# leavesnight/VIEO_SLAM

Hardware: AMD Instinct MI355X
Metric: frontend+localBA frames/sec on EuRoC MH05 stereo-VIO; ATE vs ref (higher is better)
Workload: dtype u8 (extract/match) + f64 (pose optimisation)

## Files before the change

vieo_slam_amd/csrc/orb_extractor.hip:

```cpp
#include <algorithm>
#include <cmath>
#include <type_traits>
#include <vector>

#include "../../include/vieo_orb_pattern_31.h"
#include "common.h"
#include "sincosf_exact.h"
#include "wave_ops.h"

#define QT_DEVICE
#include "quadtree.inl"

#include "orb_internal.h"

namespace vieo {

#ifndef VIEO_RESIZE_ROWS
#define VIEO_RESIZE_ROWS 32
#endif
static const int kResizeRows = VIEO_RESIZE_ROWS;
#ifndef VIEO_QT_GROUPS
#define VIEO_QT_GROUPS {1, 64}
#endif

__global__ void __launch_bounds__(256, 8)
k_resize(OrbParams P, int l, ImgSet I, const short4* __restrict__ xtab,
         const short4* __restrict__ ytab, int lds_pitch) {
  extern __shared__ __attribute__((aligned(16))) uint8_t smem[];
  const LevelDesc& D = P.lv[l];
  const int b = blockIdx.z, tid = threadIdx.x, lane = tid & 63, wave = tid >> 6;
  const int dy0 = blockIdx.y * kResizeRows, dy1 = min(dy0 + kResizeRows, D.h);
  const int dx0 = blockIdx.x * 256, dx1 = min(dx0 + 256, D.w);
  int spitch;
  const uint8_t* src = plane_ptr(P, I, b, l - 1, &spitch);
  const short4* xt = xtab + D.xtab_off;
  const short4* yt = ytab + D.ytab_off;
  const int sy_lo = yt[dy0].x, nrows = yt[dy1 - 1].y - sy_lo + 1;
  const int sx_lo = xt[dx0].x & ~3, ndw = ((xt[dx1 - 1].y + 4) >> 2) - (sx_lo >> 2);
  {
    unsigned v[12][2];
#pragma unroll
    for (int k = 0; k < 12; k++) {
      const int r = wave + 4 * k;
      const unsigned* row = (const unsigned*)(src + (size_t)(sy_lo + r) * spitch + sx_lo);
      if (r < nrows && lane < ndw) v[k][0] = row[lane];
      if (r < nrows && lane + 64 < ndw) v[k][1] = row[lane + 64];
    }
#pragma unroll
    for (int k = 0; k < 12; k++) {
      const int r = wave + 4 * k;
      if (r < nrows && lane < ndw) *(unsigned*)(smem + r * lds_pitch + 4 * lane) = v[k][0];
      if (r < nrows && lane + 64 < ndw) *(unsigned*)(smem + r * lds_pitch + 4 * (lane + 64)) = v[k][1];
    }
    for (int r = wave; r < nrows; r += 4) {
      const unsigned* row = (const unsigned*)(src + (size_t)(sy_lo + r) * spitch + sx_lo);
      for (int c = lane + (r < 48 ? 128 : 0); c < ndw; c += 64) *(unsigned*)(smem + r * lds_pitch + 4 * c) = row[c];
    }
  }
  __syncthreads();
  const int dx4 = dx0 + lane * 4;
  if (dx4 >= D.w) return;
  int x0[4], x1[4], a0[4], a1[4];
  unsigned keep = 0;
#pragma unroll
  for (int j = 0; j < 4; j++) {
    const short4 t = xt[min(dx4 + j, D.w - 1)];
    x0[j] = t.x - sx_lo, x1[j] = t.y - sx_lo, a0[j] = t.z, a1[j] = t.w;
    if (dx4 + j < D.w) keep |= 0xFFu << (8 * j);
  }
  uint8_t* dst = I.pyr + (size_t)b * I.pyr_img + D.off;
  const int wave_u = __builtin_amdgcn_readfirstlane(wave);
  for (int dy = dy0 + wave_u; dy < dy1; dy += 4) {
    const short4 y = yt[dy];
    const uint8_t* r0 = smem + (y.x - sy_lo) * lds_pitch;
    const uint8_t* r1 = smem + (y.y - sy_lo) * lds_pitch;
    const int b0 = y.z, b1 = y.w;
    unsigned out = 0;
#pragma unroll
    for (int j = 0; j < 4; j++) {
      const int h0 = r0[x0[j]] * a0[j] + r0[x1[j]] * a1[j];
      const int h1 = r1[x0[j]] * a0[j] + r1[x1[j]] * a1[j];
      const int v = (((b0 * (int)(unsigned short)(h0 >> 4)) >> 16) + ((b1 * (int)(unsigned short)(h1 >> 4)) >> 16) + 2) >> 2;
      out |= (unsigned)(v & 0xFF) << (8 * j);
    }
    *(unsigned*)(dst + (size_t)dy * D.pitch + dx4) = out & keep;
  }
}

static const int kR2W = 200, kR2H = 26, kR2Rows = 36;
__global__ void __launch_bounds__(256, 4)
k_resize2(OrbParams P, int l, ImgSet I, const short4* __restrict__ xtab, const short4* __restrict__ ytab, int lds_pitch,
          int l1_off) {
  extern __shared__ __attribute__((aligned(16))) uint8_t smem[];
  uint8_t* l1 = smem + l1_off;
  constexpr int kL1P = 260;
  const LevelDesc& D1 = P.lv[l];
  const LevelDesc& D2 = P.lv[l + 1];
  const int b = blockIdx.z, tid = threadIdx.x, lane = tid & 63, wave = tid >> 6;
  const short4* xt1 = xtab + D1.xtab_off;
  const short4* yt1 = ytab + D1.ytab_off;
  const short4* xt2 = xtab + D2.xtab_off;
  const short4* yt2 = ytab + D2.ytab_off;
  const int ex0 = blockIdx.x * kR2W, ex1 = min(ex0 + kR2W, D2.w);
  const int ey0 = blockIdx.y * kR2H, ey1 = min(ey0 + kR2H, D2.h);
  const bool last_x = ex1 == D2.w, last_y = ey1 == D2.h;
  const int rx0 = blockIdx.x == 0 ? 0 : (xt2[ex0].x & ~3), rx1 = last_x ? D1.w : min((int)xt2[ex1 - 1].y + 1, D1.w);
  const int ry0 = blockIdx.y == 0 ? 0 : (int)yt2[ey0].x, ry1 = last_y ? D1.h : min((int)yt2[ey1 - 1].y + 1, D1.h);
  const int ox1 = last_x ? D1.w : (xt2[ex1].x & ~3), oy1 = last_y ? D1.h : (int)yt2[ey1].x;
  int spitch;
  const uint8_t* src = plane_ptr(P, I, b, l - 1, &spitch);
  const int sy_lo = yt1[ry0].x, nrows = yt1[ry1 - 1].y - sy_lo + 1;
  const int sx_lo = xt1[rx0].x & ~3, ndw = ((xt1[rx1 - 1].y + 4) >> 2) - (sx_lo >> 2);
  {
    unsigned v[12][2];
#pragma unroll
    for (int k = 0; k < 12; k++) {
      const int r = wave + 4 * k;
      const unsigned* row = (const unsigned*)(src + (size_t)(sy_lo + r) * spitch + sx_lo);
      if (r < nrows && lane < ndw) v[k][0] = row[lane];
      if (r < nrows && lane + 64 < ndw) v[k][1] = row[lane + 64];
    }
#pragma unroll
    for (int k = 0; k < 12; k++) {
      const int r = wave + 4 * k;
      if (r < nrows && lane < ndw) *(unsigned*)(smem + r * lds_pitch + 4 * lane) = v[k][0];
      if (r < nrows && lane + 64 < ndw) *(unsigned*)(smem + r * lds_pitch + 4 * (lane + 64)) = v[k][1];
    }
    for (int r = wave; r < nrows; r += 4) {
      const unsigned* row = (const unsigned*)(src + (size_t)(sy_lo + r) * spitch + sx_lo);
      for (int c = lane + (r < 48 ? 128 : 0); c < ndw; c += 64) *(unsigned*)(smem + r * lds_pitch + 4 * c) = row[c];
    }
  }
  __syncthreads();
  {
    const int dx4 = rx0 + lane * 4;
    if (dx4 < rx1) {
      int x0[4], x1[4], a0[4], a1[4];
      unsigned keep = 0;
#pragma unroll
      for (int j = 0; j < 4; j++) {
        const short4 t = xt1[min(dx4 + j, D1.w - 1)];
        x0[j] = t.x - sx_lo, x1[j] = t.y - sx_lo, a0[j] = t.z, a1[j] = t.w;
        if (dx4 + j < D1.w) keep |= 0xFFu << (8 * j);
      }
      uint8_t* dst = I.pyr + (size_t)b * I.pyr_img + D1.off;
      const bool own_x = dx4 < ox1;
      const int wave_u = __builtin_amdgcn_readfirstlane(wave);
      for (int dy = ry0 + wave_u; dy < ry1; dy += 4) {
        const short4 y = yt1[dy];
        const uint8_t* r0 = smem + (y.x - sy_lo) * lds_pitch;
        const uint8_t* r1 = smem + (y.y - sy_lo) * lds_pitch;
        const int b0 = y.z, b1 = y.w;
        unsigned out = 0;
#pragma unroll
        for (int j = 0; j < 4; j++) {
          const int h0 = r0[x0[j]] * a0[j] + r0[x1[j]] * a1[j];
          const int h1 = r1[x0[j]] * a0[j] + r1[x1[j]] * a1[j];
          const int v = (((b0 * (int)(unsigned short)(h0 >> 4)) >> 16) + ((b1 * (int)(unsigned short)(h1 >> 4)) >> 16) + 2) >> 2;
          out |= (unsigned)(v & 0xFF) << (8 * j);
        }
        out &= keep;
        *(unsigned*)(l1 + (dy - ry0) * kL1P + 4 * lane) = out;
        if (own_x && dy < oy1) *(unsigned*)(dst + (size_t)dy * D1.pitch + dx4) = out;
      }
    }
  }
  __syncthreads();
  const int dx4 = ex0 + lane * 4;
  if (dx4 >= ex1) return;
  int x0[4], x1[4], a0[4], a1[4];
  unsigned keep = 0;
#pragma unroll
  for (int j = 0; j < 4; j++) {
    const short4 t = xt2[min(dx4 + j, D2.w - 1)];
    x0[j] = t.x - rx0, x1[j] = t.y - rx0, a0[j] = t.z, a1[j] = t.w;
    if (dx4 + j < D2.w) keep |= 0xFFu << (8 * j);
  }
  uint8_t* dst2 = I.pyr + (size_t)b * I.pyr_img + D2.off;
  const int wave_u = __builtin_amdgcn_readfirstlane(wave);
  for (int dy = ey0 + wave_u; dy < ey1; dy += 4) {
    const short4 y = yt2[dy];
    const uint8_t* r0 = l1 + (y.x - ry0) * kL1P;
    const uint8_t* r1 = l1 + (y.y - ry0) * kL1P;
    const int b0 = y.z, b1 = y.w;
    unsigned out = 0;
#pragma unroll
    for (int j = 0; j < 4; j++) {
      const int h0 = r0[x0[j]] * a0[j] + r0[x1[j]] * a1[j];
      const int h1 = r1[x0[j]] * a0[j] + r1[x1[j]] * a1[j];
      const int v = (((b0 * (int)(unsigned short)(h0 >> 4)) >> 16) + ((b1 * (int)(unsigned short)(h1 >> 4)) >> 16) + 2) >> 2;
      out |= (unsigned)(v & 0xFF) << (8 * j);
    }
    *(unsigned*)(dst2 + (size_t)dy * D2.pitch + dx4) = out & keep;
  }
}

#ifndef VIEO_XCD_RUN
#define VIEO_XCD_RUN 32
#endif
static const int kXcdRun = VIEO_XCD_RUN;
__device__ __forceinline__ int xcd_grouped(int bid, int G) {
  const int xcd = bid & 7, q = bid >> 3;
  return ((q / G) * 8 + xcd) * G + q % G;
}

__device__ __forceinline__ int min3i(int a, int b, int c) { return min(min(a, b), c); }
__device__ __forceinline__ int max3i(int a, int b, int c) { return max(max(a, b), c); }

__device__ __forceinline__ int fast_strength(const uint8_t* t, int p) {
  const int v = t[0];
  int d[16];
  d[0] = v - t[3 * p];
  d[1] = v - t[3 * p + 1];
  d[2] = v - t[2 * p + 2];
  d[3] = v - t[p + 3];
  d[4] = v - t[3];
  d[5] = v - t[-p + 3];
  d[6] = v - t[-2 * p + 2];
  d[7] = v - t[-3 * p + 1];
  d[8] = v - t[-3 * p];
  d[9] = v - t[-3 * p - 1];
  d[10] = v - t[-2 * p - 2];
  d[11] = v - t[-p - 3];
  d[12] = v - t[-3];
  d[13] = v - t[p - 3];
  d[14] = v - t[2 * p - 2];
  d[15] = v - t[3 * p - 1];
  int lo3[16], hi3[16];
#pragma unroll
  for (int k = 0; k < 16; k++) {
    lo3[k] = min3i(d[k], d[(k + 1) & 15], d[(k + 2) & 15]);
    hi3[k] = max3i(d[k], d[(k + 1) & 15], d[(k + 2) & 15]);
  }
  int A = -256, B = 256;
#pragma unroll
  for (int k = 0; k < 16; k++) {
    A = max(A, min3i(lo3[k], lo3[(k + 3) & 15], lo3[(k + 6) & 15]));
    B = min(B, max3i(hi3[k], hi3[(k + 3) & 15], hi3[(k + 6) & 15]));
  }
  return max(max(A, -B), 0);
}

#ifdef VIEO_FAST_STATS
__device__ unsigned long long g_fast_stats[8];
#define FAST_STAT(i, v) do { if (lane == 0) atomicAdd(&g_fast_stats[i], (unsigned long long)(v)); } while (0)
#else
#define FAST_STAT(i, v) do { } while (0)
// ... 1055 lines not shown
    }
    D.cell_end = (int)e->cells.size();
    max_ncell = std::max(max_ncell, D.cell_end - D.cell_begin);
    D.ncap = std::max(D.nfeat, 4 * D.nIni) + 8;
    ncap_max = std::max(ncap_max, D.ncap);
    D.sel_off = sel_off;
    sel_off += D.ncap;
    if (l > 0) {
      std::vector<short> t;
      D.xtab_off = (int)(xtab.size() / 4);
      resize_axis_table(P.lv[l - 1].w, D.w, true, t);
      xtab.insert(xtab.end(), t.begin(), t.end());
      D.ytab_off = (int)(ytab.size() / 4);
      resize_axis_table(P.lv[l - 1].h, D.h, false, t);
      ytab.insert(ytab.end(), t.begin(), t.end());
      const short* xt = xtab.data() + 4 * (size_t)D.xtab_off;
      const short* yt = ytab.data() + 4 * (size_t)D.ytab_off;
      for (int y0 = 0; y0 < D.h; y0 += kResizeRows)
        resize_rows = std::max(resize_rows, yt[4 * (std::min(y0 + kResizeRows, D.h) - 1) + 1] - yt[4 * y0] + 1);
      for (int x0 = 0; x0 < D.w; x0 += 256)
        resize_dw = std::max(resize_dw, ((xt[4 * (std::min(x0 + 256, D.w) - 1) + 1] + 4) >> 2) - (xt[4 * x0] >> 2));
    }
    D.tile_begin = (int)e->tiles.size();
    D.tiles_x = (D.w + kBlurTW - 1) / kBlurTW;
    for (int ty = 0; ty < (D.h + kBlurTH - 1) / kBlurTH; ty++)
      for (int tx = 0; tx < D.tiles_x; tx++) e->tiles.push_back({(short)l, (short)tx, (short)ty, 0});
    D.tile_end = (int)e->tiles.size();
  }
  P.ncells = (int)e->cells.size();
  if (max_cw - 6 > 64 || max_ch - 6 > 1023) {
    set_error("FAST cell wider than 64 pixels (image narrower than one 30-pixel cell?)");
    return VIEO_E_INVALID;
  }
  P.cell_cap = std::max(16, ((max_cw - 6 + 1) / 2) * ((max_ch - 6 + 1) / 2));
  for (int l = 0; l < e->nlevels; l++) {
    LevelDesc& D = P.lv[l];
    D.key_off = key_off;
    D.key_cap = (D.cell_end - D.cell_begin) * P.cell_cap;
    key_off += D.key_cap;
    if (D.key_cap >= (1 << 24)) {
      set_error("too many candidate keys per level");
      return VIEO_E_INVALID;
    }
  }
  P.keys_per_image = key_off;
  P.sel_per_image = sel_off;
  P.kp_cap = sel_off;
  e->ncap_max = ncap_max;
  e->scap_max = std::max(2 * ncap_max, max_ncell);
  e->pyr_img = align_up_sz(pyr_off, 256);
  e->blur_img = align_up_sz(blur_off, 256);
  e->resize_pitch = 4 * resize_dw + 4;
  e->resize_lds = resize_rows * e->resize_pitch;
  {
    bool ok = e->nlevels >= 3;
    int rows2 = 1, dw2 = 1;
    for (int l = 1; ok && l + 1 < e->nlevels; l += 2) {
      const LevelDesc &D1 = P.lv[l], &D2 = P.lv[l + 1];
      const short* xt1 = xtab.data() + 4 * (size_t)D1.xtab_off;
      const short* yt1 = ytab.data() + 4 * (size_t)D1.ytab_off;
      const short* xt2 = xtab.data() + 4 * (size_t)D2.xtab_off;
      const short* yt2 = ytab.data() + 4 * (size_t)D2.ytab_off;
      for (int ex0 = 0; ok && ex0 < D2.w; ex0 += kR2W) {
        const int ex1 = std::min(ex0 + kR2W, D2.w);
        const int rx0 = ex0 == 0 ? 0 : (xt2[4 * ex0] & ~3), rx1 = ex1 == D2.w ? D1.w : std::min(xt2[4 * (ex1 - 1) + 1] + 1, D1.w);
        const int ox1 = ex1 == D2.w ? D1.w : (xt2[4 * ex1] & ~3);
        const int ndw = ((xt1[4 * (rx1 - 1) + 1] + 4) >> 2) - ((xt1[4 * rx0] & ~3) >> 2);
        ok = rx1 - rx0 <= 256 && ox1 <= rx1 && ox1 > rx0 && ndw <= 128;
        dw2 = std::max(dw2, ndw);
      }
      for (int ey0 = 0; ok && ey0 < D2.h; ey0 += kR2H) {
        const int ey1 = std::min(ey0 + kR2H, D2.h);
        const int ry0 = ey0 == 0 ? 0 : yt2[4 * ey0], ry1 = ey1 == D2.h ? D1.h : std::min(yt2[4 * (ey1 - 1) + 1] + 1, D1.h);
        const int oy1 = ey1 == D2.h ? D1.h : yt2[4 * ey1];
        const int nrows = yt1[4 * (ry1 - 1) + 1] - yt1[4 * ry0] + 1;
        ok = ry1 - ry0 <= kR2Rows && oy1 <= ry1 && oy1 > ry0 && nrows <= 48;
        rows2 = std::max(rows2, nrows);
      }
    }
    e->resize2_ok = ok;
    e->resize2_pitch = 4 * dw2 + 4;
    e->resize2_l1_off = (rows2 * e->resize2_pitch + 15) & ~15;
    e->resize2_lds = e->resize2_l1_off + kR2Rows * 260;
  }
  e->tpitch = align_up(max_cw + 3, 4) + 4;
  e->tile_bytes = align_up(e->tpitch * max_ch, 16);
  e->score_bytes = align_up((max_cw - 4) * (max_ch - 4), 16) + 16;
  e->fast_cand_cap = std::max(256, std::min((max_cw - 6) * (max_ch - 6), 512));
  if (const char* cc = getenv("VIEO_FAST_CAND_CAP")) e->fast_cand_cap = std::max(256, atoi(cc));
  e->fast_lds = e->tile_bytes + e->score_bytes + align_up(2 * e->fast_cand_cap, 16) + 16;
  std::vector<CellPlan> plans(e->cells.size());
  for (size_t i = 0; i < e->cells.size(); i++) {
    const CellDesc& c = e->cells[i];
    const LevelDesc& D = P.lv[c.level];
    CellPlan& p = plans[i];
    memset(&p, 0, sizeof(p));
    const int x0a = c.x0 & ~3, xo = c.x0 - x0a;
    const int ndw = ((c.x0 + c.cw + 3) >> 2) - (x0a >> 2);
    if (c.level == 0) p.off = x0a, p.row = c.y0, p.pitch = 0;
    else p.off = D.off + c.y0 * D.pitch + x0a, p.row = 0, p.pitch = D.pitch;
    p.rows = c.ch | ndw << 16 | (ndw > 16 || c.ch > 64 || c.ch < 4 ? 1 << 24 : 0);
    p.tail_toff = (c.ch - 4) * e->tpitch;
    p.kbase = (3 + c.offx) | (3 + c.offy) << 12;
    const int vw = c.cw - 6, vh = c.ch - 6;
    if (vw > 0 && vh > 0) {
      const int ng = (vw + 3) >> 2, qy = 64 / ng, rx = 64 - qy * ng, m = (4096 + ng - 1) / ng;
      p.view = vw | vh << 16;
      p.align = xo | ((3 + xo) & 3) << 8 | ((3 + xo) >> 2) << 16 | ng << 24;
      p.split = qy | rx << 8 | m << 16;
      p.G = ng * vh;
      p.step_off = qy * e->tpitch + 4 * rx;
      p.wrap_off = e->tpitch - 4 * ng;
      p.Htail = (unsigned)(0x80808080ull & ((1ull << (8 * (vw - 4 * (ng - 1)))) - 1ull));
      p.clear = ((vh + 2) * (vw + 2) + 15) / 16 | (vw + 2) << 16;
    }
  }
  if (P.ncells > 1) {
    int L = 1;
    while ((1 << L) < P.ncells) L++;
    e->cell_div_mul = (unsigned)((((unsigned long long)1 << (31 + L)) + P.ncells - 1) / P.ncells);
    e->cell_div_shift = L - 1;
  } else {
    e->cell_div_mul = 0, e->cell_div_shift = 0;
  }
  e->qt_lds = 16 * e->scap_max + (4 + 16 + 4 + 4 + 4) * ncap_max + 64 + (2 * 4 + 8 + 2 * 6) * ncap_max +
              ncap_max + 64;
  int rc;
#define ENS(buf, bytes)                 \
  if ((rc = (buf).ensure(bytes)) != VIEO_OK) return rc
  ENS(e->d_pyr, e->pyr_img * B);
  if (!orb_fused()) ENS(e->d_blur, e->blur_img * B);
  ENS(e->d_cells, plans.size() * sizeof(CellPlan));
  ENS(e->d_tiles, e->tiles.size() * sizeof(BlurTile));
  ENS(e->d_xtab, std::max<size_t>(xtab.size() * 2, 8));
  ENS(e->d_ytab, std::max<size_t>(ytab.size() * 2, 8));
  ENS(e->d_cell_keys, (size_t)B * P.ncells * P.cell_cap * 4);
  ENS(e->d_cell_counts, (size_t)B * P.ncells * 4);
  ENS(e->d_keys, (size_t)B * P.keys_per_image * 4);
  ENS(e->d_kslot, (size_t)B * P.keys_per_image * 2);
  ENS(e->d_kq, (size_t)B * P.keys_per_image);
  ENS(e->d_sel, (size_t)B * P.sel_per_image * 4);
  ENS(e->d_sel_count, (size_t)B * kMaxLevels * 4);
  ENS(e->d_tmp_kp, (size_t)B * P.kp_cap * sizeof(vieo_keypoint));
  ENS(e->d_tmp_desc, (size_t)B * P.kp_cap * 32);
  ENS(e->d_tmp_counts, (size_t)B * 2 * 4);
  ENS(e->d_krec, (size_t)B * P.kp_cap * 8);
#undef ENS
  VIEO_HIP_CHECK(hipMemcpyAsync(e->d_cells.p, plans.data(), plans.size() * sizeof(CellPlan),
                                hipMemcpyHostToDevice, e->stream));
  VIEO_HIP_CHECK(hipMemcpyAsync(e->d_tiles.p, e->tiles.data(), e->tiles.size() * sizeof(BlurTile),
                                hipMemcpyHostToDevice, e->stream));
  if (!xtab.empty()) {
    VIEO_HIP_CHECK(hipMemcpyAsync(e->d_xtab.p, xtab.data(), xtab.size() * 2, hipMemcpyHostToDevice,
                                  e->stream));
    VIEO_HIP_CHECK(hipMemcpyAsync(e->d_ytab.p, ytab.data(), ytab.size() * 2, hipMemcpyHostToDevice,
                                  e->stream));
  }
  VIEO_HIP_CHECK(hipStreamSynchronize(e->stream));
  if (e->qt_lds > 64 * 1024)
    VIEO_HIP_CHECK(hipFuncSetAttribute((const void*)k_quadtree,
                                       hipFuncAttributeMaxDynamicSharedMemorySize, e->qt_lds));
  if (e->qt_lds > 160 * 1024) {
    set_error("nfeatures too large for the LDS quadtree (%d bytes)", e->qt_lds);
    return VIEO_E_INVALID;
  }
  e->w = w;
  e->h = h;
  e->B = B;
  return VIEO_OK;
}

static int run_batch(vieo_orb* e, const uint8_t* d_images, int B, int w, int h, int stride,
                     size_t image_pitch, const int* lapping, vieo_keypoint* d_kp, uint8_t* d_desc,
                     int capacity, int32_t* d_counts) {
  int rc;
  if (w != e->w || h != e->h || B > e->B) {
    if ((rc = plan_geometry(e, w, h, std::max(B, (w == e->w && h == e->h) ? e->B : 0))) != VIEO_OK)
      return rc;
  }
  if ((stride & 3) || ((uintptr_t)d_images & 3) || (image_pitch & 3)) {
    set_error("device images need 4-byte aligned base, stride and pitch");
    return VIEO_E_INVALID;
  }
  const OrbParams& P = e->P;
  ImgSet I;
  I.img0 = d_images;
  I.stride0 = stride;
  I.img_pitch = image_pitch;
  I.pyr = e->d_pyr.as<uint8_t>();
  I.pyr_img = e->pyr_img;
  I.blur = e->d_blur.as<uint8_t>();
  I.blur_img = e->blur_img;
  e->last_imgs = I;
  e->last_B = B;
  hipStream_t st = e->stream;
  Timing& T = e->tm;
  int evi = 0;
  hipEvent_t* evs = T.ev[T.steps % kTimingRing];
#define STAMP()                                                  \
  if (T.on) VIEO_HIP_CHECK(hipEventRecord(evs[evi++], st))
  STAMP();
  static const bool resize_pairs = [] {
    const char* v = getenv("VIEO_RESIZE_PAIRS");
    return !(v && atoi(v) == 0);
  }();
  for (int l = 1; l < P.nlevels;) {
    if (resize_pairs && e->resize2_ok && (l & 1) && l + 1 < P.nlevels) {
      const LevelDesc& D2 = P.lv[l + 1];
      dim3 grd((D2.w + kR2W - 1) / kR2W, (D2.h + kR2H - 1) / kR2H, B);
      hipLaunchKernelGGL(k_resize2, grd, dim3(256), e->resize2_lds, st, P, l, I, e->d_xtab.as<short4>(), e->d_ytab.as<short4>(),
                         e->resize2_pitch, e->resize2_l1_off);
      l += 2;
      continue;
    }
    const LevelDesc& D = P.lv[l];
    dim3 grd((D.w + 255) / 256, (D.h + kResizeRows - 1) / kResizeRows, B);
    hipLaunchKernelGGL(k_resize, grd, dim3(256), e->resize_lds, st, P, l, I, e->d_xtab.as<short4>(),
                       e->d_ytab.as<short4>(), e->resize_pitch);
    l++;
  }
  STAMP();
  const auto xcd_grid = [](long long items) {
    return (unsigned)((items + 8 * kXcdRun - 1) / (8 * kXcdRun) * (8 * kXcdRun));
  };
  if ((long long)P.ncells * B > 0x7FFF0000LL || (long long)e->tiles.size() * B > 0x7FFF0000LL) {
    set_error("batch too large for one launch");
    return VIEO_E_CAPACITY;
  }
  hipLaunchKernelGGL(k_fast, dim3(xcd_grid(((long long)P.ncells * B + VIEO_FAST_WAVES - 1) / VIEO_FAST_WAVES)), dim3(64 * VIEO_FAST_WAVES),
                     (size_t)align_up(e->fast_lds, 16) * VIEO_FAST_WAVES, st, I,
                     e->d_cells.as<CellPlan>(), e->d_cell_keys.as<unsigned>(), e->d_cell_counts.as<int>(),
                     e->iniTh, e->minTh, e->tpitch, e->tile_bytes, e->score_bytes, e->fast_cand_cap, P.ncells * B, P.ncells,
                     P.cell_cap, e->cell_div_mul, e->cell_div_shift, (int)align_up(e->fast_lds, 16));
  STAMP();
  {
    static const int bounds_batch[] = VIEO_QT_GROUPS;
    static const int bounds_one[] = {64};
    const bool batch = B >= 32;
    const int* bounds = batch ? bounds_batch : bounds_one;
    const size_t n_bounds = batch ? sizeof(bounds_batch) / sizeof(bounds_batch[0]) : 1;
    auto qt_caps = [&](int la, int lb, int* ncap, int* scap) {
      int nc = 1, mc = 1;
      for (int l = la; l < lb; l++) nc = std::max(nc, P.lv[l].ncap), mc = std::max(mc, P.lv[l].cell_end - P.lv[l].cell_begin);
      *ncap = nc, *scap = std::max(2 * nc, mc);
    };
    int la = 0;
    static const int qt_env = [] {
      const char* e = getenv("VIEO_QT_THREADS");
      const int v = e ? atoi(e) : 0;
      return v > 0 ? std::min(std::max(v / 64 * 64, 64), 1024) : 0;
    }();
    const int qt_threads = qt_env > 0 ? qt_env : (B <= 16 ? 512 : 256);
    for (size_t gi = 0; gi < n_bounds && la < P.nlevels; gi++) {
      const int lb = std::min(bounds[gi], P.nlevels);
      if (lb <= la) continue;
      int nc, sc;
      qt_caps(la, lb, &nc, &sc);
      const size_t lds = (size_t)16 * sc + (4 + 16 + 4 + 4 + 4) * nc + 64 + (2 * 4 + 8 + 2 * 6) * nc + nc + 64;
      hipLaunchKernelGGL(k_quadtree, dim3(lb - la, B), dim3(qt_threads), lds, st, P,
                         e->d_cell_keys.as<unsigned>(), e->d_cell_counts.as<int>(),
                         e->d_keys.as<unsigned>(), e->d_kslot.as<unsigned short>(),
                         e->d_kq.as<unsigned char>(), e->d_sel.as<unsigned>(), e->d_sel_count.as<int>(), nc, sc, la);
      la = lb;
    }
  }
  STAMP();
  const bool fused = orb_fused();
  if (!fused) {
    int rc_b = e->d_blur.ensure(e->blur_img * (size_t)e->B);
    if (rc_b != VIEO_OK) return rc_b;
    I.blur = e->d_blur.as<uint8_t>(), e->last_imgs = I;
// ... 89 lines not shown
    for (v = 0; v <= kHalfPatch; v++) e->umax[v] = 0;
    for (v = 0; v <= vmax; ++v) e->umax[v] = cv_round_d(sqrt(hp2 - v * v));
    for (v = kHalfPatch, v0 = 0; v >= vmin; --v) {
      while (e->umax[v0] == e->umax[v0 + 1]) ++v0;
      e->umax[v] = v0;
      ++v0;
    }
  }
  hipError_t he;
  {
    int lo = 0, hi = 0;
    if (priority > 0 && hipDeviceGetStreamPriorityRange(&lo, &hi) == hipSuccess && lo != hi)
      he = hipStreamCreateWithPriority(&e->stream, hipStreamNonBlocking, hi);
    else
      he = hipStreamCreateWithFlags(&e->stream, hipStreamNonBlocking);
  }
  if (he != hipSuccess) {
    set_error("hipStreamCreate: %s", hipGetErrorString(he));
    delete e;
    return VIEO_E_HIP;
  }
  std::vector<int> pat(256);
  for (int i = 0; i < 256; i++) {
    const signed char* p = VIEO_ORB_PATTERN_31 + i * 4;
    pat[i] = (int)((unsigned)(uint8_t)p[0] | ((unsigned)(uint8_t)p[1] << 8) |
                   ((unsigned)(uint8_t)p[2] << 16) | ((unsigned)(uint8_t)p[3] << 24));
  }
  if ((rc = e->d_pattern.ensure(1024)) != VIEO_OK) {
    delete e;
    return rc;
  }
  he = hipMemcpy(e->d_pattern.p, pat.data(), 1024, hipMemcpyHostToDevice);
  if (he != hipSuccess) {
    set_error("pattern upload: %s", hipGetErrorString(he));
    delete e;
    return VIEO_E_HIP;
  }
  for (auto& set : e->tm.ev)
    for (auto& ev : set) (void)hipEventCreate(&ev);
  *out = e;
  return VIEO_OK;
}

extern "C" {

void vieo_orb_destroy(vieo_orb* e) {
  if (!e) return;
  (void)hipStreamSynchronize(e->stream);
  DevBuf* bufs[] = {&e->d_pyr,   &e->d_blur,      &e->d_cells,    &e->d_tiles,      &e->d_xtab,
                    &e->d_ytab,  &e->d_cell_keys, &e->d_cell_counts, &e->d_keys,    &e->d_kslot,
                    &e->d_kq,    &e->d_sel,       &e->d_sel_count, &e->d_pattern,   &e->d_in,
                    &e->d_kp,    &e->d_desc,      &e->d_counts,   &e->d_tmp_kp,     &e->d_tmp_desc,
                    &e->d_tmp_counts, &e->d_krec,  &e->d_io,       &e->d_uright,     &e->d_depth,
                    &e->d_sad,   &e->g_start,     &e->g_rec,      &e->g_ang};
  for (DevBuf* b : bufs) b->release();
  e->h_in.release(), e->h_res.release(), e->h_io.release();
  for (auto& set : e->tm.ev)
    for (auto& ev : set)
      if (ev) (void)hipEventDestroy(ev);
  if (e->stream) (void)hipStreamDestroy(e->stream);
  delete e;
}

int vieo_orb_levels(const vieo_orb* e) { return e->nlevels; }
float vieo_orb_scale_factor(const vieo_orb* e) { return (float)e->scaleFactor; }
static int copy_tab(const std::vector<float>& v, float* out) {
  if (!out) return VIEO_E_INVALID;
  memcpy(out, v.data(), v.size() * sizeof(float));
  return VIEO_OK;
}
int vieo_orb_scale_factors(const vieo_orb* e, float* o) { return copy_tab(e->scale, o); }
int vieo_orb_inv_scale_factors(const vieo_orb* e, float* o) { return copy_tab(e->inv_scale, o); }
int vieo_orb_level_sigma2(const vieo_orb* e, float* o) { return copy_tab(e->sigma2, o); }
int vieo_orb_inv_level_sigma2(const vieo_orb* e, float* o) { return copy_tab(e->inv_sigma2, o); }
int vieo_orb_features_per_level(const vieo_orb* e, int* o) {
  if (!o) return VIEO_E_INVALID;
  memcpy(o, e->feats.data(), e->feats.size() * sizeof(int));
  return VIEO_OK;
}
int vieo_orb_max_keypoints(const vieo_orb* e) {
  int s = 0;
  for (int l = 0; l < e->nlevels; l++) s += std::max(e->feats[l], 16) + 8;
  return s;
}

int vieo_orb_extract_batch_device(vieo_orb* e, const uint8_t* d_images, int n_images, int width,
                                  int height, int stride, size_t image_pitch_bytes,
                                  const int* h_lapping, vieo_keypoint* d_keypoints,
                                  uint8_t* d_descriptors, int capacity, int32_t* d_counts) {
  if (!e || !d_images || n_images <= 0 || !d_keypoints || !d_descriptors || !d_counts ||
      capacity <= 0) {
    set_error("vieo_orb_extract_batch_device: invalid arguments");
    return VIEO_E_INVALID;
  }
  if (width <= 0 || height <= 0) return VIEO_E_EMPTY;
  return run_batch(e, d_images, n_images, width, height, stride, image_pitch_bytes, h_lapping,
                   d_keypoints, d_descriptors, capacity, d_counts);
}

#ifdef VIEO_FAST_STATS
int vieo_fast_stats(unsigned long long* out8) {
  unsigned long long z[8] = {0};
  VIEO_HIP_CHECK(hipDeviceSynchronize());
  VIEO_HIP_CHECK(hipMemcpyFromSymbol(out8, HIP_SYMBOL(vieo::g_fast_stats), sizeof(z)));
  VIEO_HIP_CHECK(hipMemcpyToSymbol(HIP_SYMBOL(vieo::g_fast_stats), z, sizeof(z)));
  return VIEO_OK;
}
// ... 233 lines not shown
```

vieo_slam_amd/csrc/orb_internal.h:

```cpp
#pragma once
#include <vector>

#include "common.h"

namespace vieo {

static const int kPatchSize = 31, kHalfPatch = 15, kEdge = 19;
static const int kMaxLevels = 16;
#ifndef VIEO_BLUR_TH
#define VIEO_BLUR_TH 96
#endif
static const int kBlurTW = 64, kBlurTH = VIEO_BLUR_TH;

struct LevelDesc {
  int w, h, pitch, off;
  int boff;
  int cell_begin, cell_end;
  int nfeat;
  int regW, regH, nIni;
  float hX;
  int key_off, key_cap;
  int sel_off, ncap;
  int xtab_off, ytab_off;
  float scale;
// ... 3 lines not shown

struct OrbParams {
  int nlevels, cell_cap, ncells, keys_per_image, sel_per_image, kp_cap;
  int umax[kHalfPatch + 1];
  LevelDesc lv[kMaxLevels];
};

struct CellDesc {
  short level, x0, y0, cw, ch, offx, offy, pad;
};

struct alignas(16) CellPlan {
  int off;
  int row;
  int pitch;
  int rows;
  int view;
  int align;
  int split;
  int G;
  int step_off, wrap_off;
  unsigned Htail;
  int clear;
  int kbase;
  int tail_toff;
  int pad0, pad1;
};
static_assert(sizeof(CellPlan) == 64, "CellPlan is one 64-byte scalar load");

struct ImgSet {
  const uint8_t* img0;
  int stride0;
  size_t img_pitch;
  uint8_t* pyr;
  size_t pyr_img;
  uint8_t* blur;
  size_t blur_img;
};

__device__ __forceinline__ const uint8_t* plane_ptr(const OrbParams& P, const ImgSet& I, int b,
                                                    int l, int* pitch) {
  if (l == 0) {
    *pitch = I.stride0;
    return I.img0 + (size_t)b * I.img_pitch;
  }
  *pitch = P.lv[l].pitch;
  return I.pyr + (size_t)b * I.pyr_img + P.lv[l].off;
}

struct BlurTile {
  short level, tx, ty, pad;
};

static const int kTimingRing = 64;
struct Timing {
  bool on = false;
  hipEvent_t ev[kTimingRing][VIEO_ORB_NSTAGES] = {};
  long steps = 0;
};

int orb_create_with_priority(vieo_orb** out, int nfeatures, float scale_factor, int nlevels, int ini_th, int min_th, int priority);

}

struct vieo_orb {
  int nfeatures, nlevels, iniTh, minTh;
  double scaleFactor;
  std::vector<float> scale, inv_scale, sigma2, inv_sigma2;
  std::vector<int> feats;
  int umax[vieo::kHalfPatch + 1];
  hipStream_t stream = nullptr;
  int w = 0, h = 0, B = 0;
  vieo::OrbParams P;
  std::vector<vieo::CellDesc> cells;
  std::vector<vieo::BlurTile> tiles;
  unsigned cell_div_mul = 0;
  int cell_div_shift = 0;
  int tpitch = 0, fast_cand_cap = 0, tile_bytes = 0, score_bytes = 0, fast_lds = 0, qt_lds = 0, ncap_max = 0, scap_max = 0;
  int resize_pitch = 0, resize_lds = 0;
  int resize2_pitch = 0, resize2_l1_off = 0, resize2_lds = 0;
  bool resize2_ok = false;
  size_t pyr_img = 0, blur_img = 0;
  vieo::DevBuf d_pyr, d_blur, d_cells, d_tiles, d_xtab, d_ytab, d_cell_keys, d_cell_counts, d_keys,
      d_kslot, d_kq, d_sel, d_sel_count, d_pattern, d_in, d_kp, d_desc, d_counts, d_tmp_kp,
      d_tmp_desc, d_tmp_counts, d_krec;
  int out_cap = 0;
  int last_B = 0;
  vieo::ImgSet last_imgs{};
  vieo::Timing tm;
  vieo::PinnedBuf h_in, h_res, h_io;
  vieo::DevBuf d_io;
  unsigned long long epoch = 0;
  int res_n = -1, res_mono = 0;
  vieo_keypoint res_sample[16];
  vieo::DevBuf d_uright, d_depth, d_sad;
  unsigned long long uright_epoch = ~0ull;
  std::vector<float> uright_host;
  vieo::DevBuf g_start, g_rec, g_ang;
  unsigned long long grid_epoch = ~0ull;
};
```

Measured before the change: 62120.

## Software-pipeline resize taps, precompute tile spans, and XCD-swizzle resize grids

```diff
diff --git a/vieo_slam_amd/csrc/orb_extractor.hip b/vieo_slam_amd/csrc/orb_extractor.hip
--- a/vieo_slam_amd/csrc/orb_extractor.hip
+++ b/vieo_slam_amd/csrc/orb_extractor.hip
@@ -23,37 +23,116 @@
 #define VIEO_QT_GROUPS {1, 64}
 #endif
 
+__device__ __forceinline__ int resize_row(int first, int end, int k) { return max(min(first + 4 * k, end - 1), 0); }
+template <int K>
+struct RowTaps {
+  int lo[K], hi[K];
+};
+template <int K>
+__device__ __forceinline__ void row_taps_load(RowTaps<K>& y, const short4* __restrict__ yt, int first, int end) {
+#pragma unroll
+  for (int k = 0; k < K; k++) {
+    const int2 e = ((const int2*)yt)[resize_row(first, end, k)];
+    y.lo[k] = e.x, y.hi[k] = e.y;
+  }
+}
+template <int K>
+__device__ __forceinline__ void row_taps_pin(RowTaps<K>& y) {
+#pragma unroll
+  for (int k = 0; k < K; k++) asm volatile("" : "+s"(y.lo[k]), "+s"(y.hi[k]));
+}
+template <int K, class Emit>
+__device__ __forceinline__ void resize_rows(const RowTaps<K>& y, int first, int end, const uint8_t* S, int pitch, int row_lo,
+                                            const int (&x0)[4], const int (&x1)[4], const int (&a0)[4], const int (&a1)[4],
+                                            Emit emit) {
+  int t[3][8];
+  const auto taps = [&](int s, int(&q)[8]) {
+    const int k = s >> 1, j0 = 2 * (s & 1);
+    const uint8_t* r0 = S + ((int)(short)y.lo[k] - row_lo) * pitch;
+    const uint8_t* r1 = S + ((y.lo[k] >> 16) - row_lo) * pitch;
+#pragma unroll
+    for (int j = 0; j < 2; j++)
+      q[4 * j] = r0[x0[j0 + j]], q[4 * j + 1] = r0[x1[j0 + j]], q[4 * j + 2] = r1[x0[j0 + j]], q[4 * j + 3] = r1[x1[j0 + j]];
+  };
+  taps(0, t[0]);
+  taps(1, t[1]);
+  unsigned out = 0;
+#pragma unroll
+  for (int s = 0; s < 2 * K; s++) {
+    const int k = s >> 1, j0 = 2 * (s & 1);
+    if (s + 2 < 2 * K) taps(s + 2, t[(s + 2) % 3]);
+    __builtin_amdgcn_sched_barrier(0);
+    const int(&q)[8] = t[s % 3];
+    const int b0 = (short)y.hi[k], b1 = y.hi[k] >> 16;
+#pragma unroll
+    for (int j = 0; j < 2; j++) {
+      const int h0 = q[4 * j] * a0[j0 + j] + q[4 * j + 1] * a1[j0 + j];
+      const int h1 = q[4 * j + 2] * a0[j0 + j] + q[4 * j + 3] * a1[j0 + j];
+      const int v = (((b0 * (int)(unsigned short)(h0 >> 4)) >> 16) + ((b1 * (int)(unsigned short)(h1 >> 4)) >> 16) + 2) >> 2;
+      out |= (unsigned)(v & 0xFF) << (8 * (j0 + j));
+    }
+    if (j0) emit(k, resize_row(first, end, k), out), out = 0;
+  }
+}
+
+__device__ __forceinline__ bool resize_tile(int ntx, int nty, int B, int* bx, int* by, int* b) {
+  const int gid = blockIdx.x, xcd = gid & 7, q = gid >> 3, T = ntx * nty;
+  const int tile = q % T;
+  *b = (q / T) * 8 + xcd;
+  *bx = tile % ntx, *by = tile / ntx;
+  return *b < B;
+}
+static unsigned resize_grid(int ntx, int nty, int B) { return 8u * (unsigned)(ntx * nty) * (unsigned)((B + 7) / 8); }
+
+struct Band {
+  unsigned v[12][2];
+};
+__device__ __forceinline__ void band_load(Band& B, const uint8_t* src, int spitch, int sy_lo, int sx_lo, int nrows, int ndw,
+                                          int lane, int wave) {
+#pragma unroll
+  for (int k = 0; k < 12; k++) {
+    const int r = wave + 4 * k;
+    const unsigned* row = (const unsigned*)(src + (size_t)(sy_lo + r) * spitch + sx_lo);
+    if (r < nrows && lane < ndw) B.v[k][0] = row[lane];
+    if (r < nrows && lane + 64 < ndw) B.v[k][1] = row[lane + 64];
+  }
+}
+__device__ __forceinline__ void band_store(const Band& B, uint8_t* smem, int lds_pitch, int nrows, int ndw, int lane, int wave) {
+#pragma unroll
+  for (int k = 0; k < 12; k++) {
+    const int r = wave + 4 * k;
+    if (r < nrows && lane < ndw) *(unsigned*)(smem + r * lds_pitch + 4 * lane) = B.v[k][0];
+    if (r < nrows && lane + 64 < ndw) *(unsigned*)(smem + r * lds_pitch + 4 * (lane + 64)) = B.v[k][1];
+  }
+}
+
 __global__ void __launch_bounds__(256, 8)
 k_resize(OrbParams P, int l, ImgSet I, const short4* __restrict__ xtab,
-         const short4* __restrict__ ytab, int lds_pitch) {
+         const short4* __restrict__ ytab, int lds_pitch, int ntx, int nty, int B) {
   extern __shared__ __attribute__((aligned(16))) uint8_t smem[];
   const LevelDesc& D = P.lv[l];
-  const int b = blockIdx.z, tid = threadIdx.x, lane = tid & 63, wave = tid >> 6;
-  const int dy0 = blockIdx.y * kResizeRows, dy1 = min(dy0 + kResizeRows, D.h);
-  const int dx0 = blockIdx.x * 256, dx1 = min(dx0 + 256, D.w);
+  int bx, by, b;
+  if (!resize_tile(ntx, nty, B, &bx, &by, &b)) return;
+  const int tid = threadIdx.x, lane = tid & 63, wave = tid >> 6;
+  const int wave_u = __builtin_amdgcn_readfirstlane(wave);
+  const int dy0 = by * kResizeRows, dy1 = min(dy0 + kResizeRows, D.h);
+  const int dx0 = bx * 256, dx1 = min(dx0 + 256, D.w);
   int spitch;
   const uint8_t* src = plane_ptr(P, I, b, l - 1, &spitch);
   const short4* xt = xtab + D.xtab_off;
   const short4* yt = ytab + D.ytab_off;
   const int sy_lo = yt[dy0].x, nrows = yt[dy1 - 1].y - sy_lo + 1;
   const int sx_lo = xt[dx0].x & ~3, ndw = ((xt[dx1 - 1].y + 4) >> 2) - (sx_lo >> 2);
+  RowTaps<(kResizeRows + 3) / 4> y;
+  row_taps_load(y, yt, dy0 + wave_u, dy1);
   {
-    unsigned v[12][2];
-#pragma unroll
-    for (int k = 0; k < 12; k++) {
-      const int r = wave + 4 * k;
-      const unsigned* row = (const unsigned*)(src + (size_t)(sy_lo + r) * spitch + sx_lo);
-      if (r < nrows && lane < ndw) v[k][0] = row[lane];
-      if (r < nrows && lane + 64 < ndw) v[k][1] = row[lane + 64];
-    }
-#pragma unroll
-    for (int k = 0; k < 12; k++) {
-      const int r = wave + 4 * k;
-      if (r < nrows && lane < ndw) *(unsigned*)(smem + r * lds_pitch + 4 * lane) = v[k][0];
-      if (r < nrows && lane + 64 < ndw) *(unsigned*)(smem + r * lds_pitch + 4 * (lane + 64)) = v[k][1];
-    }
+    Band B;
+    band_load(B, src, spitch, sy_lo, sx_lo, nrows, ndw, lane, wave_u);
+    row_taps_pin(y);
+    band_store(B, smem, lds_pitch, nrows, ndw, lane, wave_u);
     for (int r = wave; r < nrows; r += 4) {
       const unsigned* row = (const unsigned*)(src + (size_t)(sy_lo + r) * spitch + sx_lo);
+#pragma unroll 1
       for (int c = lane + (r < 48 ? 128 : 0); c < ndw; c += 64) *(unsigned*)(smem + r * lds_pitch + 4 * c) = row[c];
     }
   }
@@ -69,99 +148,77 @@
     if (dx4 + j < D.w) keep |= 0xFFu << (8 * j);
   }
   uint8_t* dst = I.pyr + (size_t)b * I.pyr_img + D.off;
-  const int wave_u = __builtin_amdgcn_readfirstlane(wave);
-  for (int dy = dy0 + wave_u; dy < dy1; dy += 4) {
-    const short4 y = yt[dy];
-    const uint8_t* r0 = smem + (y.x - sy_lo) * lds_pitch;
-    const uint8_t* r1 = smem + (y.y - sy_lo) * lds_pitch;
-    const int b0 = y.z, b1 = y.w;
-    unsigned out = 0;
-#pragma unroll
-    for (int j = 0; j < 4; j++) {
-      const int h0 = r0[x0[j]] * a0[j] + r0[x1[j]] * a1[j];
-      const int h1 = r1[x0[j]] * a0[j] + r1[x1[j]] * a1[j];
-      const int v = (((b0 * (int)(unsigned short)(h0 >> 4)) >> 16) + ((b1 * (int)(unsigned short)(h1 >> 4)) >> 16) + 2) >> 2;
-      out |= (unsigned)(v & 0xFF) << (8 * j);
-    }
-    *(unsigned*)(dst + (size_t)dy * D.pitch + dx4) = out & keep;
-  }
-}
-
-static const int kR2W = 200, kR2H = 26, kR2Rows = 36;
-__global__ void __launch_bounds__(256, 4)
-k_resize2(OrbParams P, int l, ImgSet I, const short4* __restrict__ xtab, const short4* __restrict__ ytab, int lds_pitch,
-          int l1_off) {
+  const int dpitch = D.pitch;
+  resize_rows(y, dy0 + wave_u, dy1, smem, lds_pitch, sy_lo, x0, x1, a0, a1, [&](int, int dy, unsigned out) {
+    *(unsigned*)(dst + (unsigned)(dy * dpitch + dx4)) = out & keep;
+  });
+}
+
+static const int kR2W = 200, kR2H = 28, kR2Rows = 36;
+__global__ void __launch_bounds__(256, 5)
+k_resize2(OrbParams P, int l, ImgSet I, const short4* __restrict__ xtab, const short4* __restrict__ ytab,
+          const R2Span* __restrict__ cols, const R2Span* __restrict__ rows, int lds_pitch, int l1_off, int tw, int th,
+          int ntx, int nty, int B) {
   extern __shared__ __attribute__((aligned(16))) uint8_t smem[];
   uint8_t* l1 = smem + l1_off;
   constexpr int kL1P = 260;
+  constexpr int K1 = (kR2Rows + 3) / 4, K2 = (kR2H + 3) / 4;
   const LevelDesc& D1 = P.lv[l];
   const LevelDesc& D2 = P.lv[l + 1];
-  const int b = blockIdx.z, tid = threadIdx.x, lane = tid & 63, wave = tid >> 6;
+  int bx, by, b;
+  if (!resize_tile(ntx, nty, B, &bx, &by, &b)) return;
+  const int tid = threadIdx.x, lane = tid & 63, wave = tid >> 6;
+  const int wave_u = __builtin_amdgcn_readfirstlane(wave);
   const short4* xt1 = xtab + D1.xtab_off;
   const short4* yt1 = ytab + D1.ytab_off;
   const short4* xt2 = xtab + D2.xtab_off;
   const short4* yt2 = ytab + D2.ytab_off;
-  const int ex0 = blockIdx.x * kR2W, ex1 = min(ex0 + kR2W, D2.w);
-  const int ey0 = blockIdx.y * kR2H, ey1 = min(ey0 + kR2H, D2.h);
-  const bool last_x = ex1 == D2.w, last_y = ey1 == D2.h;
-  const int rx0 = blockIdx.x == 0 ? 0 : (xt2[ex0].x & ~3), rx1 = last_x ? D1.w : min((int)xt2[ex1 - 1].y + 1, D1.w);
-  const int ry0 = blockIdx.y == 0 ? 0 : (int)yt2[ey0].x, ry1 = last_y ? D1.h : min((int)yt2[ey1 - 1].y + 1, D1.h);
-  const int ox1 = last_x ? D1.w : (xt2[ex1].x & ~3), oy1 = last_y ? D1.h : (int)yt2[ey1].x;
+  struct Span {
+    int r0, r1, o1, s_lo, n;
+  };
+  const auto span = [](const R2Span& s) { return Span{s.r0, s.r1, s.o1, s.s_lo, s.n}; };
+  const Span C = span(cols[bx]), R = span(rows[by]);
+  const int ex0 = bx * tw, ex1 = min(ex0 + tw, D2.w);
+  const int ey0 = by * th, ey1 = min(ey0 + th, D2.h);
+  RowTaps<K1> ya;
+  RowTaps<K2> yb;
+  row_taps_load(ya, yt1, R.r0 + wave_u, R.r1);
+  row_taps_load(yb, yt2, ey0 + wave_u, ey1);
   int spitch;
   const uint8_t* src = plane_ptr(P, I, b, l - 1, &spitch);
-  const int sy_lo = yt1[ry0].x, nrows = yt1[ry1 - 1].y - sy_lo + 1;
-  const int sx_lo = xt1[rx0].x & ~3, ndw = ((xt1[rx1 - 1].y + 4) >> 2) - (sx_lo >> 2);
   {
-    unsigned v[12][2];
-#pragma unroll
-    for (int k = 0; k < 12; k++) {
-      const int r = wave + 4 * k;
-      const unsigned* row = (const unsigned*)(src + (size_t)(sy_lo + r) * spitch + sx_lo);
-      if (r < nrows && lane < ndw) v[k][0] = row[lane];
-      if (r < nrows && lane + 64 < ndw) v[k][1] = row[lane + 64];
-    }
-#pragma unroll
-    for (int k = 0; k < 12; k++) {
-      const int r = wave + 4 * k;
-      if (r < nrows && lane < ndw) *(unsigned*)(smem + r * lds_pitch + 4 * lane) = v[k][0];
-      if (r < nrows && lane + 64 < ndw) *(unsigned*)(smem + r * lds_pitch + 4 * (lane + 64)) = v[k][1];
-    }
-    for (int r = wave; r < nrows; r += 4) {
-      const unsigned* row = (const unsigned*)(src + (size_t)(sy_lo + r) * spitch + sx_lo);
-      for (int c = lane + (r < 48 ? 128 : 0); c < ndw; c += 64) *(unsigned*)(smem + r * lds_pitch + 4 * c) = row[c];
-    }
+    Band B;
+    band_load(B, src, spitch, R.s_lo, C.s_lo, R.n, C.n, lane, wave_u);
+    row_taps_pin(ya);
+    row_taps_pin(yb);
+    band_store(B, smem, lds_pitch, R.n, C.n, lane, wave_u);
   }
   __syncthreads();
   {
-    const int dx4 = rx0 + lane * 4;
-    if (dx4 < rx1) {
+    const int dx4 = C.r0 + lane * 4;
+    if (dx4 < C.r1) {
       int x0[4], x1[4], a0[4], a1[4];
       unsigned keep = 0;
 #pragma unroll
       for (int j = 0; j < 4; j++) {
         const short4 t = xt1[min(dx4 + j, D1.w - 1)];
-        x0[j] = t.x - sx_lo, x1[j] = t.y - sx_lo, a0[j] = t.z, a1[j] = t.w;
+        x0[j] = t.x - C.s_lo, x1[j] = t.y - C.s_lo, a0[j] = t.z, a1[j] = t.w;
         if (dx4 + j < D1.w) keep |= 0xFFu << (8 * j);
       }
+      const int ry0 = R.r0, ry1 = R.r1;
+      unsigned outs[K1];
+      resize_rows(ya, ry0 + wave_u, ry1, smem, lds_pitch, R.s_lo, x0, x1, a0, a1, [&](int k, int dy, unsigned out) {
+        outs[k] = out & keep;
+        *(unsigned*)(l1 + (dy - ry0) * kL1P + 4 * lane) = outs[k];
+      });
       uint8_t* dst = I.pyr + (size_t)b * I.pyr_img + D1.off;
-      const bool own_x = dx4 < ox1;
-      const int wave_u = __builtin_amdgcn_readfirstlane(wave);
-      for (int dy = ry0 + wave_u; dy < ry1; dy += 4) {
-        const short4 y = yt1[dy];
-        const uint8_t* r0 = smem + (y.x - sy_lo) * lds_pitch;
-        const uint8_t* r1 = smem + (y.y - sy_lo) * lds_pitch;
-        const int b0 = y.z, b1 = y.w;
-        unsigned out = 0;
-#pragma unroll
-        for (int j = 0; j < 4; j++) {
-          const int h0 = r0[x0[j]] * a0[j] + r0[x1[j]] * a1[j];
-          const int h1 = r1[x0[j]] * a0[j] + r1[x1[j]] * a1[j];
-          const int v = (((b0 * (int)(unsigned short)(h0 >> 4)) >> 16) + ((b1 * (int)(unsigned short)(h1 >> 4)) >> 16) + 2) >> 2;
-          out |= (unsigned)(v & 0xFF) << (8 * j);
+      const int pitch1 = D1.pitch, oy1 = R.o1;
+      if (dx4 < C.o1) {
+#pragma unroll
+        for (int k = 0; k < K1; k++) {
+          const int dy = ry0 + wave_u + 4 * k;
+          if (dy < min(oy1, ry1)) *(unsigned*)(dst + (unsigned)(dy * pitch1 + dx4)) = outs[k];
         }
-        out &= keep;
-        *(unsigned*)(l1 + (dy - ry0) * kL1P + 4 * lane) = out;
-        if (own_x && dy < oy1) *(unsigned*)(dst + (size_t)dy * D1.pitch + dx4) = out;
       }
     }
   }
@@ -173,26 +230,14 @@
 #pragma unroll
   for (int j = 0; j < 4; j++) {
     const short4 t = xt2[min(dx4 + j, D2.w - 1)];
-    x0[j] = t.x - rx0, x1[j] = t.y - rx0, a0[j] = t.z, a1[j] = t.w;
+    x0[j] = t.x - C.r0, x1[j] = t.y - C.r0, a0[j] = t.z, a1[j] = t.w;
     if (dx4 + j < D2.w) keep |= 0xFFu << (8 * j);
   }
   uint8_t* dst2 = I.pyr + (size_t)b * I.pyr_img + D2.off;
-  const int wave_u = __builtin_amdgcn_readfirstlane(wave);
-  for (int dy = ey0 + wave_u; dy < ey1; dy += 4) {
-    const short4 y = yt2[dy];
-    const uint8_t* r0 = l1 + (y.x - ry0) * kL1P;
-    const uint8_t* r1 = l1 + (y.y - ry0) * kL1P;
-    const int b0 = y.z, b1 = y.w;
-    unsigned out = 0;
-#pragma unroll
-    for (int j = 0; j < 4; j++) {
-      const int h0 = r0[x0[j]] * a0[j] + r0[x1[j]] * a1[j];
-      const int h1 = r1[x0[j]] * a0[j] + r1[x1[j]] * a1[j];
-      const int v = (((b0 * (int)(unsigned short)(h0 >> 4)) >> 16) + ((b1 * (int)(unsigned short)(h1 >> 4)) >> 16) + 2) >> 2;
-      out |= (unsigned)(v & 0xFF) << (8 * j);
-    }
-    *(unsigned*)(dst2 + (size_t)dy * D2.pitch + dx4) = out & keep;
-  }
+  const int pitch2 = D2.pitch;
+  resize_rows(yb, ey0 + wave_u, ey1, l1, kL1P, R.r0, x0, x1, a0, a1, [&](int, int dy, unsigned out) {
+    *(unsigned*)(dst2 + (unsigned)(dy * pitch2 + dx4)) = out & keep;
+  });
 }
 
 #ifndef VIEO_XCD_RUN
@@ -1354,7 +1399,12 @@
   e->blur_img = align_up_sz(blur_off, 256);
   e->resize_pitch = 4 * resize_dw + 4;
   e->resize_lds = resize_rows * e->resize_pitch;
+  std::vector<R2Span> r2span;
   {
+    static const bool balance = [] {
+      const char* v = getenv("VIEO_RESIZE_BALANCE");
+      return !(v && atoi(v) == 0);
+    }();
     bool ok = e->nlevels >= 3;
     int rows2 = 1, dw2 = 1;
     for (int l = 1; ok && l + 1 < e->nlevels; l += 2) {
@@ -1363,22 +1413,40 @@
       const short* yt1 = ytab.data() + 4 * (size_t)D1.ytab_off;
       const short* xt2 = xtab.data() + 4 * (size_t)D2.xtab_off;
       const short* yt2 = ytab.data() + 4 * (size_t)D2.ytab_off;
-      for (int ex0 = 0; ok && ex0 < D2.w; ex0 += kR2W) {
-        const int ex1 = std::min(ex0 + kR2W, D2.w);
+      vieo_orb::Resize2Pair& R = e->resize2_pair[l / 2];
+      const int nx = (D2.w + kR2W - 1) / kR2W;
+      R.tw = balance ? align_up((D2.w + nx - 1) / nx, 4) : kR2W;
+      R.ntx = (D2.w + R.tw - 1) / R.tw;
+      R.col_off = (int)r2span.size();
+      for (int ex0 = 0; ok && ex0 < D2.w; ex0 += R.tw) {
+        const int ex1 = std::min(ex0 + R.tw, D2.w);
         const int rx0 = ex0 == 0 ? 0 : (xt2[4 * ex0] & ~3), rx1 = ex1 == D2.w ? D1.w : std::min(xt2[4 * (ex1 - 1) + 1] + 1, D1.w);
         const int ox1 = ex1 == D2.w ? D1.w : (xt2[4 * ex1] & ~3);
-        const int ndw = ((xt1[4 * (rx1 - 1) + 1] + 4) >> 2) - ((xt1[4 * rx0] & ~3) >> 2);
+        const int sx_lo = xt1[4 * rx0] & ~3, ndw = ((xt1[4 * (rx1 - 1) + 1] + 4) >> 2) - (sx_lo >> 2);
         ok = rx1 - rx0 <= 256 && ox1 <= rx1 && ox1 > rx0 && ndw <= 128;
         dw2 = std::max(dw2, ndw);
+        r2span.push_back({rx0, rx1, ox1, sx_lo, ndw, {0, 0, 0}});
       }
-      for (int ey0 = 0; ok && ey0 < D2.h; ey0 += kR2H) {
-        const int ey1 = std::min(ey0 + kR2H, D2.h);
-        const int ry0 = ey0 == 0 ? 0 : yt2[4 * ey0], ry1 = ey1 == D2.h ? D1.h : std::min(yt2[4 * (ey1 - 1) + 1] + 1, D1.h);
-        const int oy1 = ey1 == D2.h ? D1.h : yt2[4 * ey1];
-        const int nrows = yt1[4 * (ry1 - 1) + 1] - yt1[4 * ry0] + 1;
-        ok = ry1 - ry0 <= kR2Rows && oy1 <= ry1 && oy1 > ry0 && nrows <= 48;
-        rows2 = std::max(rows2, nrows);
-      }
+      R.row_off = (int)r2span.size();
+      const auto rows_fit = [&](int th) {
+        r2span.resize(R.row_off);
+        int tallest = 1;
+        for (int ey0 = 0; ey0 < D2.h; ey0 += th) {
+          const int ey1 = std::min(ey0 + th, D2.h);
+          const int ry0 = ey0 == 0 ? 0 : yt2[4 * ey0], ry1 = ey1 == D2.h ? D1.h : std::min(yt2[4 * (ey1 - 1) + 1] + 1, D1.h);
+          const int oy1 = ey1 == D2.h ? D1.h : yt2[4 * ey1];
+          const int sy_lo = yt1[4 * ry0], nrows = yt1[4 * (ry1 - 1) + 1] - sy_lo + 1;
+          if (!(ry1 - ry0 <= kR2Rows && oy1 <= ry1 && oy1 > ry0 && nrows <= 48)) return 0;
+          tallest = std::max(tallest, nrows);
+          r2span.push_back({ry0, ry1, oy1, sy_lo, nrows, {0, 0, 0}});
+        }
+        return tallest;
+      };
+      int tallest = 0;
+      for (R.th = kR2H & ~3; ok && !(tallest = rows_fit(R.th)) && R.th > 4;) R.th -= 4;
+      ok = ok && tallest > 0;
+      rows2 = std::max(rows2, tallest);
+      R.nty = (D2.h + R.th - 1) / R.th;
     }
     e->resize2_ok = ok;
     e->resize2_pitch = 4 * dw2 + 4;
@@ -1436,6 +1504,7 @@
   ENS(e->d_tiles, e->tiles.size() * sizeof(BlurTile));
   ENS(e->d_xtab, std::max<size_t>(xtab.size() * 2, 8));
   ENS(e->d_ytab, std::max<size_t>(ytab.size() * 2, 8));
+  ENS(e->d_r2span, std::max<size_t>(r2span.size() * sizeof(R2Span), 32));
   ENS(e->d_cell_keys, (size_t)B * P.ncells * P.cell_cap * 4);
   ENS(e->d_cell_counts, (size_t)B * P.ncells * 4);
   ENS(e->d_keys, (size_t)B * P.keys_per_image * 4);
@@ -1458,6 +1527,9 @@
     VIEO_HIP_CHECK(hipMemcpyAsync(e->d_ytab.p, ytab.data(), ytab.size() * 2, hipMemcpyHostToDevice,
                                   e->stream));
   }
+  if (!r2span.empty())
+    VIEO_HIP_CHECK(hipMemcpyAsync(e->d_r2span.p, r2span.data(), r2span.size() * sizeof(R2Span), hipMemcpyHostToDevice,
+                                  e->stream));
   VIEO_HIP_CHECK(hipStreamSynchronize(e->stream));
   if (e->qt_lds > 64 * 1024)
     VIEO_HIP_CHECK(hipFuncSetAttribute((const void*)k_quadtree,
@@ -1508,17 +1580,18 @@
   }();
   for (int l = 1; l < P.nlevels;) {
     if (resize_pairs && e->resize2_ok && (l & 1) && l + 1 < P.nlevels) {
-      const LevelDesc& D2 = P.lv[l + 1];
-      dim3 grd((D2.w + kR2W - 1) / kR2W, (D2.h + kR2H - 1) / kR2H, B);
-      hipLaunchKernelGGL(k_resize2, grd, dim3(256), e->resize2_lds, st, P, l, I, e->d_xtab.as<short4>(), e->d_ytab.as<short4>(),
-                         e->resize2_pitch, e->resize2_l1_off);
+      const vieo_orb::Resize2Pair& R = e->resize2_pair[l / 2];
+      const R2Span* spans = e->d_r2span.as<R2Span>();
+      hipLaunchKernelGGL(k_resize2, dim3(resize_grid(R.ntx, R.nty, B)), dim3(256), e->resize2_lds, st, P, l, I,
+                         e->d_xtab.as<short4>(), e->d_ytab.as<short4>(), spans + R.col_off, spans + R.row_off, e->resize2_pitch,
+                         e->resize2_l1_off, R.tw, R.th, R.ntx, R.nty, B);
       l += 2;
       continue;
     }
     const LevelDesc& D = P.lv[l];
-    dim3 grd((D.w + 255) / 256, (D.h + kResizeRows - 1) / kResizeRows, B);
-    hipLaunchKernelGGL(k_resize, grd, dim3(256), e->resize_lds, st, P, l, I, e->d_xtab.as<short4>(),
-                       e->d_ytab.as<short4>(), e->resize_pitch);
+    const int ntx = (D.w + 255) / 256, nty = (D.h + kResizeRows - 1) / kResizeRows;
+    hipLaunchKernelGGL(k_resize, dim3(resize_grid(ntx, nty, B)), dim3(256), e->resize_lds, st, P, l, I, e->d_xtab.as<short4>(),
+                       e->d_ytab.as<short4>(), e->resize_pitch, ntx, nty, B);
     l++;
   }
   STAMP();
@@ -1714,7 +1787,7 @@
                     &e->d_kq,    &e->d_sel,       &e->d_sel_count, &e->d_pattern,   &e->d_in,
                     &e->d_kp,    &e->d_desc,      &e->d_counts,   &e->d_tmp_kp,     &e->d_tmp_desc,
                     &e->d_tmp_counts, &e->d_krec,  &e->d_io,       &e->d_uright,     &e->d_depth,
-                    &e->d_sad,   &e->g_start,     &e->g_rec,      &e->g_ang};
+                    &e->d_sad,   &e->g_start,     &e->g_rec,      &e->g_ang,        &e->d_r2span};
   for (DevBuf* b : bufs) b->release();
   e->h_in.release(), e->h_res.release(), e->h_io.release();
   for (auto& set : e->tm.ev)
diff --git a/vieo_slam_amd/csrc/orb_internal.h b/vieo_slam_amd/csrc/orb_internal.h
--- a/vieo_slam_amd/csrc/orb_internal.h
+++ b/vieo_slam_amd/csrc/orb_internal.h
@@ -79,6 +79,11 @@
   short level, tx, ty, pad;
 };
 
+struct alignas(32) R2Span {
+  int r0, r1, o1, s_lo, n, pad[3];
+};
+static_assert(sizeof(R2Span) == 32, "R2Span is one 32-byte scalar load");
+
 static const int kTimingRing = 64;
 struct Timing {
   bool on = false;
@@ -107,10 +112,14 @@
   int resize_pitch = 0, resize_lds = 0;
   int resize2_pitch = 0, resize2_l1_off = 0, resize2_lds = 0;
   bool resize2_ok = false;
+  struct Resize2Pair {
+    int tw, th, ntx, nty, col_off, row_off;
+  } resize2_pair[vieo::kMaxLevels / 2] = {};
   size_t pyr_img = 0, blur_img = 0;
   vieo::DevBuf d_pyr, d_blur, d_cells, d_tiles, d_xtab, d_ytab, d_cell_keys, d_cell_counts, d_keys,
       d_kslot, d_kq, d_sel, d_sel_count, d_pattern, d_in, d_kp, d_desc, d_counts, d_tmp_kp,
-      d_tmp_desc, d_tmp_counts, d_krec;
+      d_tmp_desc, d_tmp_counts, d_krec,
+      d_r2span;
   int out_cap = 0;
   int last_B = 0;
   vieo::ImgSet last_imgs{};
```

Result: no change. 62070 (-0.1%).
